# aarchiiive/diff-unet-amos

Measured on AMD Instinct MI355X. Metric: denoised voxel-steps/sec on 96^3 16-class AMOS patches, higher is better.
Workload: dtype f16

## Files before the change

diff_unet_amos_amd/csrc/conv3_args.hpp:

```cpp
#pragma once
#include "common.hpp"

namespace dua {

struct Conv3Args {
  const void* x; const void* w; const float* bias; void* y;
  stat_t* stats;
  InXform xf;
  int N, D, H, W;
  int Cin, Cin_stride, Cin_off;
  int Cout, Cout_stride, Cout_off;
  int nchunks, ntiles, tiles_h, tiles_w, cout_pad;
  int ksplit, units_per_split;
  float* part;
  int tap_ch;
  int in_blk, out_blk;
  const void* bw_raw; int bw_stride, bw_off;
  InXform bw_xf;
  double* bw_sums;
};

int launch_conv3_wide(Conv3Args a, int D, hipStream_t s, bool persistent, int stagger = 0);
bool conv3_wide_takes_bwd_sums(const Conv3Args& a);

}
```

diff_unet_amos_amd/csrc/conv3d_igemm.hip:

```cpp
#include "common.hpp"
#include "../../include/dua_hip.h"
#include "conv3_args.hpp"
#include "stamp.hpp"
#include <algorithm>

namespace dua {

namespace c3 {
constexpr int TD = 4, TH = 8, TW = 8;
constexpr int HD = TD + 2, HH = TH + 2, HW = TW + 2;
constexpr int KG = 4;
constexpr int VS = KG * 16;
constexpr int RS = HW * VS + 16;
constexpr int PS = HH * RS;
constexpr int HALO_BYTES = HD * PS;
constexpr int BN = 64;
}

static inline int conv_variant_of(const dua_conv3_desc* d) { return d->policy & 0xff; }
static inline bool conv_policy_ok(const dua_conv3_desc* d) {
  const int v = d->policy & 0xff;
  return (d->policy & ~(0xff | DUA_POLICY_NO_FINISH)) == 0 && (v == 0 || v == 2 || v == 3 || v == 6 || v == 7 || v == 8 || v == 9);
}

#ifdef DUA_ABLATE
extern int g_wgrad_abl;
#endif

namespace c3v2 {
using namespace c3;
constexpr int SLAB = 3 * KG * BN * 16;
constexpr int LDS_MAIN = HALO_BYTES + 2 * SLAB;
}

__device__ __forceinline__ void glds16(const void* g, void* lds_wave_base) {
  __builtin_amdgcn_global_load_lds((const __attribute__((address_space(1))) void*)g,
                                   (__attribute__((address_space(3))) void*)lds_wave_base, 16, 0, 0);
}

template <typename T, int TDP = 4, int NKS = 2, bool HALF = false, bool BIG = false>
__global__ __launch_bounds__(256, BIG ? 1 : 2) void conv3d_k3_v2_kernel(Conv3Args a) {
  using namespace c3v2;
  constexpr int TD = TDP, HD = TDP + 2, MB = TDP == 2 ? 1 : 2;
  constexpr int NW = 4, NTHR = 64 * NW;
  constexpr int BSLAB = 3 * SLAB;
  constexpr int HALO_BYTES = HD * PS, LDS_MAIN = HALO_BYTES + (BIG ? 3 * BSLAB : 2 * SLAB);
  static_assert(!BIG || (NKS == 2 && !HALF), "the kd-plane form is the plain 32-channel-chunk kernel");
  constexpr int NITEMS = HD * HH * HW * KG, NIT = (NITEMS + NTHR - 1) / NTHR;
  constexpr int NPIECE = SLAB / 16, NSL = (NPIECE + NTHR - 1) / NTHR;
  using Frag = typename Elem<T>::Frag;
  constexpr int EPG = Elem<T>::EPG;
  constexpr int CK = KG * EPG;
  extern __shared__ __attribute__((aligned(16))) char smem[];
  char* halo = smem;
  char* wbuf = smem + HALO_BYTES;
  float* xsc = (float*)(smem + LDS_MAIN);
  float* xsh = xsc + a.nchunks * CK;
  float* xad = xsh + a.nchunks * CK;

  const int tid = threadIdx.x, lane = tid & 63, wave = tid >> 6;
  const int r = lane & 31, hh = lane >> 5;
  const int dwave = TDP == 2 ? wave >> 1 : wave;
  const int hbase = TDP == 2 ? (wave & 1) * 4 : 0;
  const int tile = xcd_remap(blockIdx.x, a.ntiles);
  const int ct = blockIdx.y, n = blockIdx.z % a.N;
  const int tw_ = tile % a.tiles_w, th_ = (tile / a.tiles_w) % a.tiles_h, td_ = tile / (a.tiles_w * a.tiles_h);
  const int d0 = td_ * TD, h0 = th_ * TH, w0 = tw_ * TW;
  const bool fused = a.xf.stats != nullptr;

  const int kg_t = tid & (KG - 1);
  long goff[NIT]; int loff[NIT];
  const T* xin = (const T*)a.x + (long)n * a.D * a.H * a.W * a.Cin_stride + a.Cin_off;
#pragma unroll
  for (int j = 0; j < NIT; ++j) {
    int it = tid + NTHR * j;
// ... 710 lines not shown
#pragma unroll
      for (int e = 0; e < 4; ++e) {
        o[e] = (T)acc[e];
        const float f = (float)o[e];
        s[e] += f; q[e] += (part_t)f * (part_t)f;
      }
      if (c < Cout) {
        T* yp = y + ((long)n * vox + v) * Cout_stride + Cout_off + c;
#pragma unroll
        for (int e = 0; e < 4; ++e) yp[e] = o[e];
      }
    }
  }
#pragma unroll
  for (int e = 0; e < 4; ++e) { red[threadIdx.x][e] = s[e]; red[threadIdx.x][4 + e] = q[e]; }
  __syncthreads();
  for (int ch = threadIdx.x; ch < 4 * G; ch += 256) {
    const int g4 = ch >> 2, e = ch & 3;
    double S = 0, Q = 0;
    for (int j = 0; j < VL; ++j) { S += (double)red[j * G + g4][e]; Q += (double)red[j * G + g4][4 + e]; }
    if (ch < Cout) stats_add(stats, n, cout_pad, blockIdx.x & (STAT_REPLICAS - 1), ch, S, Q);
  }
}


static inline void choose_split(int base_wgs, int units, int* ksplit, int* ups, int target = 320, int max_base = 64) {
  *ksplit = 1; *ups = units;
  if (base_wgs > max_base || units <= 1) return;
  int want = target == 320 ? (320 + base_wgs - 1) / base_wgs : target / base_wgs;
  if (want < 1) want = 1;
  if (want > units) want = units;
  *ups = (units + want - 1) / want;
  *ksplit = (units + *ups - 1) / *ups;
}

constexpr int PARTIAL_LDS_PAD = 36 * 1024;

static const LdsAttr kConvLdsAttrs[] = {
    {(const void*)conv3d_k3_v2_kernel<f16, 4>, c3v2::LDS_MAIN + 3 * 4 * 1024 + PARTIAL_LDS_PAD},
    {(const void*)conv3d_k3_v2_kernel<float, 4>, c3v2::LDS_MAIN + 3 * 4 * 1024 + PARTIAL_LDS_PAD},
    {(const void*)conv3d_k3_v2_kernel<f16, 4, 1>, c3v2::LDS_MAIN + 4096 + PARTIAL_LDS_PAD},
    {(const void*)conv3d_k3_v2_kernel<f16, 4, 0>, c3v2::LDS_MAIN + 4096 + PARTIAL_LDS_PAD},
    {(const void*)conv3d_k3_v2_kernel<f16, 4, 2, true>, c3v2::LDS_MAIN + 3 * 4 * 1024 + PARTIAL_LDS_PAD},
    {(const void*)conv3d_k3_first_kernel, c3f::LDS_F + 2048 + PARTIAL_LDS_PAD},
    {(const void*)conv3d_k3_v2_kernel<f16, 2>, c3v2::LDS_MAIN + 3 * 4 * 1024},
    {(const void*)conv3d_k3_v2_kernel<float, 2>, c3v2::LDS_MAIN + 3 * 4 * 1024},
    {(const void*)conv3d_k3_v2_kernel<f16, 4, 2, false, true>, 160 * 1024},
    {(const void*)conv3d_k3_v2_kernel<float, 4, 2, false, true>, 160 * 1024},
    {(const void*)conv3d_k3_v2_kernel<f16, 2, 2, false, true>, 160 * 1024},
    {(const void*)conv3d_k3_v2_kernel<float, 2, 2, false, true>, 160 * 1024},
};
static const LdsAttrs kConvLdsReg(kConvLdsAttrs);

static int conv3_kernel_kind(const dua_conv3_desc* d, bool fused) {
  const int g_conv_variant = conv_variant_of(d);
  if (d->dtype != DUA_F16) return 0;
  if (d->tap_channel_plus1 > 0) return (d->tap_channel_plus1 == 17 && g_conv_variant == 0) ? 1 : 0;
  const long tiles = (long)((d->D + 3) / 4) * ((d->H + 7) / 8) * ((d->W + 7) / 8) * ((d->Cout + c3::BN - 1) / c3::BN) * d->N;
  const long vox = (long)d->D * d->H * d->W;
  if ((g_conv_variant == 0 || g_conv_variant == 8 || g_conv_variant == 9) && !d->background && tiles >= 1024 && d->D % 8 == 0 && d->H % 8 == 0 && d->W % 8 == 0 &&
      d->Cin % 16 == 0 && d->Cin <= (fused ? 256 : 384) && vox * d->Cin_stride < 0x7fffffffL)
    return 2;
  return 0;
}

struct BwdSums { const void* raw; int stride, off; const dua_in_norm* in; double* sums; };

template <typename T>
static int launch_conv3(const dua_conv3_desc* d, const void* x, const void* w, const float* bias,
                        const dua_in_norm* in, void* y, stat_t* stats, float* ws, long ws_bytes, hipStream_t s,
                        const BwdSums* bw = nullptr) {
  using namespace c3;
  constexpr int CK = KG * Elem<T>::EPG;
  Conv3Args a;
  a.x = x; a.w = w; a.bias = bias; a.y = y; a.stats = stats;
  a.bw_raw = nullptr; a.bw_stride = a.bw_off = 0; a.bw_xf = make_xform(nullptr, d->Cout); a.bw_sums = nullptr;
  if (bw) {
    a.bw_raw = bw->raw; a.bw_stride = bw->stride; a.bw_off = bw->off; a.bw_xf = make_xform(bw->in, d->Cout); a.bw_sums = bw->sums;
  }
  a.xf = make_xform(in, d->Cin);
  a.N = d->N; a.D = d->D; a.H = d->H; a.W = d->W;
  a.Cin = d->Cin; a.Cin_stride = d->Cin_stride; a.Cin_off = d->Cin_off;
  a.Cout = d->Cout; a.Cout_stride = d->Cout_stride; a.Cout_off = d->Cout_off;
  a.nchunks = (d->Cin + CK - 1) / CK;
  const int td = (d->D + TD - 1) / TD;
  a.tiles_h = (d->H + TH - 1) / TH; a.tiles_w = (d->W + TW - 1) / TW;
  a.ntiles = td * a.tiles_h * a.tiles_w;
  const int nct = (d->Cout + BN - 1) / BN;
  a.cout_pad = nct * BN;
  a.ksplit = 1; a.units_per_split = a.nchunks * 3; a.part = nullptr; a.tap_ch = -1;
  a.in_blk = d->layout & DUA_IN_BLOCKED ? 1 : 0; a.out_blk = d->layout & DUA_OUT_BLOCKED ? 1 : 0;
  if (a.nchunks * CK > 1024 || !conv_policy_ok(d)) return DUA_ERR_ARG;
  const int g_conv_variant = conv_variant_of(d);
  const int kind = conv3_kernel_kind(d, in && in->stats);
  if ((a.in_blk && kind != 2) || (a.out_blk && kind == 0)) return DUA_ERR_ARG;
  if ((a.in_blk && (d->Cin_off % 16 || d->Cin_stride % 16)) || (a.out_blk && (d->Cout_off % 16 || d->Cout_stride % 16))) return DUA_ERR_ARG;
  const int xf_bytes = in && in->stats ? 3 * 4 * a.nchunks * CK : 0;
  if (int e = ensure_prepared()) return e;
  const long vox = (long)d->D * d->H * d->W;
  const int bg_pad = d->background ? PARTIAL_LDS_PAD : 0;
  if (d->tap_channel_plus1 > 0) {
    a.tap_ch = d->tap_channel_plus1 - 1;
    if constexpr (sizeof(T) != 2) return DUA_ERR_ARG;
    else {
      if (a.nchunks != 1 || (in && in->stats) || (a.tap_ch != 0 && a.tap_ch != 16) || d->Cin != a.tap_ch + 8) return DUA_ERR_ARG;
      dim3 grid(a.ntiles, nct, d->N);
      if (kind == 1) {
        const int cus = device_cus();
        if (cus <= 0) return DUA_ERR_ARG;
        const int items = a.ntiles * d->N;
        const int wgs = std::max(1, (bg_pad ? 1 : 2) * cus / nct);
        hipLaunchKernelGGL(conv3d_k3_first_kernel, dim3(std::min(items, wgs), nct, 1), dim3(256), c3f::LDS_F + 2048 + bg_pad, s, a, items);
        return (int)hipGetLastError();
      }
      if (a.tap_ch == 16) hipLaunchKernelGGL((conv3d_k3_v2_kernel<T, 4, 1>), grid, dim3(256), c3v2::LDS_MAIN + 4096 + bg_pad, s, a);
      else hipLaunchKernelGGL((conv3d_k3_v2_kernel<T, 4, 0>), grid, dim3(256), c3v2::LDS_MAIN + 4096 + bg_pad, s, a);
      return (int)hipGetLastError();
    }
  }
  if constexpr (sizeof(T) == 2) {
    if (kind == 2) return launch_conv3_wide(a, d->D, s, g_conv_variant >= 8, g_conv_variant == 9 ? 2 : 0);
  }
  if (bw) return DUA_ERR_ARG;
  const bool autop = g_conv_variant == 0 || g_conv_variant == 2 || g_conv_variant == 6 || g_conv_variant == 7 || g_conv_variant >= 8;
  const bool big = g_conv_variant == 0 || g_conv_variant == 2 || g_conv_variant == 7 || g_conv_variant >= 8;
  if (ws != nullptr && autop) {
    int ks, ups;
    if (g_conv_variant == 2) choose_split(a.ntiles * nct * d->N, a.nchunks * 3, &ks, &ups, 512, 256);
    else choose_split(a.ntiles * nct * d->N, a.nchunks * 3, &ks, &ups, big ? 256 : 320);
    if (ks > 1 && (long)ks * d->N * vox * a.cout_pad * 4 <= ws_bytes) { a.ksplit = ks; a.units_per_split = ups; a.part = ws; }
  }
  if (a.ksplit == 1 && ((autop && a.ntiles * nct * d->N < 200 && a.ntiles * nct * d->N > 64) || g_conv_variant == 3)) {
    const int td2 = (d->D + 1) / 2;
    a.ntiles = td2 * a.tiles_h * a.tiles_w;
    dim3 grid2(a.ntiles, nct, d->N);
    constexpr int LDS2 = 4 * c3::HH * c3::RS + 2 * c3v2::SLAB;
    const bool big2 = big && (long)a.ntiles * nct * d->N <= 256;
    if (big2) hipLaunchKernelGGL((conv3d_k3_v2_kernel<T, 2, 2, false, true>), grid2, dim3(256), 4 * c3::HH * c3::RS + 9 * c3v2::SLAB + xf_bytes, s, a);
    else hipLaunchKernelGGL((conv3d_k3_v2_kernel<T, 2>), grid2, dim3(256), LDS2 + xf_bytes, s, a);
    return (int)hipGetLastError();
  }
  dim3 grid(a.ntiles, nct, d->N * a.ksplit);
  if (a.ksplit > 1) {
    if (big) hipLaunchKernelGGL((conv3d_k3_v2_kernel<T, 4, 2, false, true>), grid, dim3(256), c3::HALO_BYTES + 9 * c3v2::SLAB + xf_bytes, s, a);
    else hipLaunchKernelGGL(conv3d_k3_v2_kernel<T>, grid, dim3(256), c3v2::LDS_MAIN + xf_bytes, s, a);
    if (d->policy & DUA_POLICY_NO_FINISH) return (int)hipGetLastError();
    const int G = a.cout_pad / 4 > 256 ? 256 : a.cout_pad / 4;
    if (a.cout_pad / 4 > 256) return DUA_ERR_ARG;
    const int VL = 256 / G;
    int ITER = 8;
    while (ITER > 1 && (vox + (long)VL * ITER - 1) / ((long)VL * ITER) < 128) ITER >>= 1;
    dim3 fgrid((unsigned)((vox + (long)VL * ITER - 1) / ((long)VL * ITER)), d->N);
    hipLaunchKernelGGL(splitk_finish_kernel<T>, fgrid, dim3(256), 0, s, (const float*)ws, a.ksplit, d->N, vox, a.cout_pad,
                       d->Cout, bias, (T*)y, d->Cout_stride, d->Cout_off, stats, G, VL, ITER);
    return (int)hipGetLastError();
  }
  if (sizeof(T) == 2 && d->Cin - (a.nchunks - 1) * CK <= CK / 2)
    hipLaunchKernelGGL((conv3d_k3_v2_kernel<T, 4, 2, true>), grid, dim3(256), c3v2::LDS_MAIN + xf_bytes + bg_pad, s, a);
  else
    hipLaunchKernelGGL(conv3d_k3_v2_kernel<T>, grid, dim3(256), c3v2::LDS_MAIN + xf_bytes + bg_pad, s, a);
  return (int)hipGetLastError();
}

}

extern "C" {

#ifdef DUA_STAMP
long dua_debug_stamps(void* host, long bytes) { return dua::stamps_out(host, bytes); }
#endif

#ifdef DUA_ABLATE
int dua_set_option(int key, int value) {
  if (key == 3 && value >= 0 && value < 16) { dua::g_wgrad_abl = value; return 0; }
  return DUA_ERR_ARG;
}
#endif

int dua_conv3d_k3_kernel_kind(const dua_conv3_desc* d, int fused, int has_workspace) {
  if (!d || !dua::conv_policy_ok(d)) return DUA_ERR_ARG;
  (void)has_workspace;
  return dua::conv3_kernel_kind(d, fused != 0);
}

long dua_conv3d_k3_workspace(const dua_conv3_desc* d) {
  using namespace dua::c3;
  if (!d || (d->dtype != DUA_F16 && d->dtype != DUA_F32)) return DUA_ERR_ARG;
  const int ck = 4 * (d->dtype == DUA_F16 ? 8 : 4);
  const int nch = (d->Cin + ck - 1) / ck, nct = (d->Cout + BN - 1) / BN;
  const int tiles = ((d->D + TD - 1) / TD) * ((d->H + TH - 1) / TH) * ((d->W + TW - 1) / TW);
  int ks, ups;
  dua::choose_split(tiles * nct * d->N, nch * 3, &ks, &ups);
  return ks > 1 ? (long)ks * d->N * d->D * d->H * d->W * nct * BN * 4 : 0;
}

int dua_conv3d_k3_fwd(const dua_conv3_desc* d, const void* x, const void* w_packed, const float* bias_padded,
                      const dua_in_norm* in, void* y, dua_stat_word* out_stats, void* workspace, long workspace_bytes,
                      void* stream) {
  if (!d || !x || !w_packed || !bias_padded || !y || !out_stats) return DUA_ERR_ARG;
  if (d->Cin % 8 || d->Cout % 8 || d->Cin_stride % 8 || d->Cout_stride % 8 || d->Cin_off % 8 || d->Cout_off % 8)
    return DUA_ERR_ARG;
  if (in && in->stats && (!in->gamma || !in->beta || in->c_pad < d->Cin || in->count <= 0 || !(in->slope >= 0.f && in->slope <= 1.f))) return DUA_ERR_ARG;
  if (d->dtype == DUA_F16)
    return dua::launch_conv3<dua::f16>(d, x, w_packed, bias_padded, in, y, out_stats, (float*)workspace, workspace_bytes, (hipStream_t)stream);
  if (d->dtype == DUA_F32)
    return dua::launch_conv3<float>(d, x, w_packed, bias_padded, in, y, out_stats, (float*)workspace, workspace_bytes, (hipStream_t)stream);
  return DUA_ERR_ARG;
}

int dua_conv3d_k3_dgrad_reduce_supported(const dua_conv3_desc* d) {
  if (!d || d->dtype != DUA_F16 || d->layout || d->tap_channel_plus1 || d->background || dua::conv_variant_of(d) != 0) return 0;
  return dua::conv3_kernel_kind(d, false) == 2 ? 1 : 0;
}

int dua_conv3d_k3_dgrad_reduce(const dua_conv3_desc* d, const void* dy, const void* w_packed, const float* bias_padded, void* dx,
                               const void* raw, int raw_stride, int raw_off, const dua_in_norm* raw_in, double* sums, void* stream) {
  if (!dua_conv3d_k3_dgrad_reduce_supported(d) || !dy || !w_packed || !bias_padded || !dx || !raw || !raw_in || !sums) return DUA_ERR_ARG;
  if (d->Cin % 8 || d->Cout % 8 || d->Cin_stride % 8 || d->Cout_stride % 8 || d->Cin_off % 8 || d->Cout_off % 8) return DUA_ERR_ARG;
  if (!raw_in->stats || !raw_in->gamma || !raw_in->beta || raw_in->c_pad < d->Cout || raw_in->count <= 0 ||
      !(raw_in->slope >= 0.f && raw_in->slope <= 1.f) || raw_stride % 8 || raw_off % 8 || raw_off + d->Cout > raw_stride)
    return DUA_ERR_ARG;
  const dua::BwdSums bw{raw, raw_stride, raw_off, raw_in, sums};
  return dua::launch_conv3<dua::f16>(d, dy, w_packed, bias_padded, nullptr, dx, nullptr, nullptr, 0, (hipStream_t)stream, &bw);
}

}
```

diff_unet_amos_amd/csrc/conv3d_wide.hip:

```cpp
#include "common.hpp"
#include "../../include/dua_hip.h"
#include "conv3_args.hpp"
#include "stamp.hpp"
#include "named_acc.hpp"

namespace dua {

namespace c3w {
constexpr int TH = 8, TW = 8, HH = TH + 2, HW = TW + 2;
constexpr int VSF = 32, RSF = 12 * VSF, PSF = HH * RSF;
constexpr int BN = 64;
constexpr int WPLANE = 18 * 1024;
constexpr int HALO_MAX = 10 * PSF;
constexpr int LDS_FIXED = HALO_MAX + 2 * WPLANE;
constexpr int SLAB = 3 * 4 * BN * 16;
}

__device__ __forceinline__ void dma_piece(const char* src_lane, unsigned lds_dst) {
  unsigned keep;
  asm volatile("s_mov_b32 %0, m0\n\ts_mov_b32 m0, %2\n\ts_nop 0\n\tglobal_load_lds_dwordx4 %1, off\n\ts_mov_b32 m0, %0"
               : "=&s"(keep) : "v"(src_lane), "s"(__builtin_amdgcn_readfirstlane(lds_dst)) : "memory");
}

#ifndef WIDE_LA
#define WIDE_LA 1
#endif
template <int MB, bool BWD = false>
__device__ __forceinline__ void wide_tile(const Conv3Args& a, char* smem, const int d0, const int h0, const int w0,
                                          const int ct, const int n, const int replica) {
  using namespace c3w;
  using T = f16;
  constexpr int TD = 2 * MB, HD = TD + 2, NH = MB / 2;
  char* halo = smem;
  char* wbuf = smem + HALO_MAX;
  float* xsc = (float*)(smem + LDS_FIXED);
  float* xsh = xsc + a.Cin;
  float* xad = xsh + a.Cin;

  const int tid = threadIdx.x, lane = tid & 63, wave = tid >> 6;
  const int r = lane & 31, hh = lane >> 5;
  const bool fused = a.xf.stats != nullptr;
  const int nhc = (a.Cin + 15) >> 4;
  const int U = nhc * 3;

  const int p_t = tid & 1, pos = tid >> 1;
  const int hy = pos / HW, hx = pos - hy * HW;
  const int gh = h0 + hy - 1, gw = w0 + hx - 1;
  const bool ok_hw = pos < HH * HW && (unsigned)gh < (unsigned)a.H && (unsigned)gw < (unsigned)a.W;
  const int vstride = a.in_blk ? 16 : a.Cin_stride;
  const long hcstride = a.in_blk ? (long)a.D * a.H * a.W * 16 : 16;
  const T* xin = (const T*)a.x + (long)n * a.D * a.H * a.W * a.Cin_stride + (a.in_blk ? (long)(a.Cin_off >> 4) * a.D * a.H * a.W * 16 : a.Cin_off) + p_t * 8;
  const int voff = ok_hw ? (((d0 - 1) * a.H + gh) * a.W + gw) * vstride : 0;
  const int pstep = a.H * a.W * vstride;
  const int loff = pos < HH * HW ? hy * RSF + hx * VSF + ((p_t ^ (hy & 1)) << 4) : HW * VSF + (p_t << 4);
  f16x8 hreg[HD];
  auto load_halo = [&](int hc, int j0, int j1) {
    const T* src = xin + hc * hcstride;
#pragma unroll
    for (int j = 0; j < HD; ++j) {
      if (j < j0 || j >= j1) continue;
      const bool dok = (unsigned)(d0 + j - 1) < (unsigned)a.D;
      hreg[j] = *(const f16x8*)(src + (ok_hw && dok ? voff + j * pstep : 0));
    }
  };
  auto store_halo = [&](int hc) {
    float sc[8], sh[8], ad[8], sn[8];
    if (fused) {
      const int c0 = hc * 16 + p_t * 8;
#pragma unroll
      for (int e = 0; e < 8; ++e) { sc[e] = xsc[c0 + e]; sh[e] = xsh[c0 + e]; ad[e] = xad[c0 + e]; }
      xform_prep<T>(sc, sh, ad, sn, a.xf.slope);
    }
#pragma unroll
    for (int j = 0; j < HD; ++j) {
      f16x8 v = hreg[j];
      if (fused) v = xform_frag<T>(v, sc, sh, ad, sn, a.xf.slope);
      const f32x4 raw = __builtin_bit_cast(f32x4, v);
      const bool ok = ok_hw && (unsigned)(d0 + j - 1) < (unsigned)a.D;
      f32x4 o;
#pragma unroll
      for (int e = 0; e < 4; ++e) o[e] = ok ? raw[e] : 0.f;
      *(f32x4*)(halo + loff + j * PSF) = o;
    }
  };

  const char* wsrc = (const char*)a.w + (long)ct * a.nchunks * 9 * SLAB + lane * 16;
  const unsigned wlds = (unsigned)(size_t)(__attribute__((address_space(3))) char*)wbuf;
  auto dma_plane = [&](int u, int slot) {
    const int hc = u / 3, kd = u - hc * 3;
    const char* src = wsrc + (long)((hc >> 1) * 3 + kd) * 3 * SLAB + (hc & 1) * 2048;
#pragma unroll
    for (int j = 0; j < 5; ++j) {
      const int p = wave + 4 * j;
      if (p < 18) dma_piece(src + ((p >> 1) * 4 + (p & 1)) * 1024, wlds + slot * WPLANE + p * 1024);
    }
  };

  DUA_STAMP_AT(0, true);
  DUA_STAMP_AT(2, false);
  float bias_q[2];
#pragma unroll
  for (int q = 0; q < 2; ++q) {
    const int bc = ct * BN + q * 32 + r;
    bias_q[q] = bc >= a.Cout ? 0.f : a.bias[bc];
  }
  constexpr int UN = 4;
  stat_t sv[UN][2 * STAT_WORDS];
  float gam[UN], bet[UN], addv[UN];
  if (fused) {
    const int part = lane >> 4;
#pragma unroll
    for (int u = 0; u < UN; ++u) {
      const int c = (wave + 4 * u) * 16 + (lane & 15), cc = c < a.Cin ? c : a.Cin - 1;
      gam[u] = a.xf.gamma[cc]; bet[u] = a.xf.beta[cc];
      addv[u] = a.xf.add ? a.xf.add[(long)n * a.xf.add_stride + cc] : 0.f;
      const stat_t* sp = a.xf.stats + ((long)n * STAT_REPLICAS + 2 * part) * STAT_WORDS * a.xf.c_pad + cc;
      if ((wave + 4 * u) * 16 < a.Cin) {
#pragma unroll
        for (int k = 0; k < 2 * STAT_WORDS; ++k) sv[u][k] = sp[(long)k * a.xf.c_pad];
      } else {
#pragma unroll
        for (int k = 0; k < 2 * STAT_WORDS; ++k) sv[u][k] = 0;
      }
    }
  }
  float* bwc = (float*)(smem + LDS_FIXED) + (fused ? 3 * a.Cin : 0);
  double bwS = 0, bwQ = 0;
  float bwg = 0.f, bwb = 0.f;
  constexpr bool bwd = BWD;
  if (bwd) {
    const int c = ct * BN + wave * 16 + (lane & 15), cc = c < a.Cout ? c : a.Cout - 1;
    bwg = a.bw_xf.gamma[cc]; bwb = a.bw_xf.beta[cc];
    stats_read_wave16(a.bw_xf.stats, n, a.bw_xf.c_pad, cc, bwS, bwQ);
  }
  DUA_STAMP_AT(56, false);
  load_halo(0, 0, HD);
  DUA_STAMP_AT(57, false);
  dma_plane(0, 0);
  DUA_STAMP_AT(59, false);
  if (fused) {
    const int part = lane >> 4;
    double Sm = 0, Qm = 0;
    float gm = 0.f, bm = 0.f, am = 0.f;
#pragma unroll
    for (int u = 0; u < UN; ++u) {
      stat_t w[STAT_WORDS];
#pragma unroll
      for (int k = 0; k < STAT_WORDS; ++k) {
        w[k] = sv[u][k] + sv[u][STAT_WORDS + k];
        w[k] += __shfl_xor(w[k], 16);
        w[k] += __shfl_xor(w[k], 32);
      }
      if (part == u) {
        Sm = (double)w[0] + (double)w[1] * (1.0 / STAT_FRAC);
        Qm = (double)w[2] + (double)w[3] * (1.0 / STAT_FRAC);
        gm = gam[u]; bm = bet[u]; am = addv[u];
      }
    }
    const int c = (wave + 4 * part) * 16 + (lane & 15);
    const double mean = Sm * a.xf.inv_count;
    double var = Qm * a.xf.inv_count - mean * mean;
    var = var > 0 ? var : 0;
    const float g = gm * (float)(1.0 / sqrt(var + (double)a.xf.eps));
    if (c < a.Cin) {
      xsc[c] = g;
      xsh[c] = bm - (float)mean * g;
      xad[c] = am;
    }
    __syncthreads();
  }
  if (bwd && lane < 16) {
    const double mean = bwS * a.bw_xf.inv_count;
    double var = bwQ * a.bw_xf.inv_count - mean * mean;
    var = var > 0 ? var : 0;
    const int cl = wave * 16 + lane;
    bwc[cl] = (float)mean;
    bwc[64 + cl] = (float)(1.0 / sqrt(var + (double)a.bw_xf.eps));
    bwc[128 + cl] = bwg;
    bwc[192 + cl] = bwb;
  }
  DUA_STAMP_AT(60, false);
  DUA_STAMP_AT(61, false);
  store_halo(0);
  const int dsl = MB == 4 ? 2 * wave : wave;
  f32x16 acc[MB][2];
#pragma unroll
  for (int q = 0; q < 2; ++q)
#pragma unroll
    for (int m = 0; m < MB; ++m)
#pragma unroll
      for (int i = 0; i < 16; ++i) acc[m][q][i] = bias_q[q];
  asm volatile("s_waitcnt vmcnt(0)" ::: "memory");
  __syncthreads();
  DUA_STAMP_AT(3, false);

  const int sw = (r >> 3) & 1;
  const int a_base = dsl * PSF + (r >> 3) * RSF + (r & 7) * VSF;
  const int a_even = a_base + ((hh ^ sw) << 4), a_odd = a_base + ((hh ^ sw ^ 1) << 4);
  const int b_base = (hh * BN + r) * 16;

  auto phase = [&](int kd, int slot) __attribute__((always_inline)) {
    const char* hp = halo + kd * PSF;
    const char* wb = wbuf + slot * WPLANE + b_base;
    f16x8 fa[WIDE_LA + 1][2], fb[2][2];
    auto ldA = [&](int t, int sub, int b) {
      const int kh = t / 3, kw = t - kh * 3;
      const char* ap = hp + ((kh & 1) ? a_odd : a_even) + sub * PSF + kh * RSF + kw * VSF;
      fa[b][0] = *(const f16x8*)ap;
      fa[b][1] = *(const f16x8*)(ap + 4 * RSF);
    };
    auto ldB = [&](int t, int b) {
      fb[b][0] = *(const f16x8*)(wb + t * 2048);
      fb[b][1] = *(const f16x8*)(wb + t * 2048 + 512);
    };
    ldB(0, 0);
#pragma unroll
    for (int h = 0; h < WIDE_LA; ++h) ldA(h / NH, h % NH, h);
#pragma unroll
    for (int h = 0; h < 9 * NH; ++h) {
      const int t = h / NH, sub = h % NH;
      if (h + WIDE_LA < 9 * NH) {
        const int t1 = (h + WIDE_LA) / NH, sub1 = (h + WIDE_LA) % NH;
        if (WIDE_LA == 1 && sub1 == 0) ldB(t1, t1 & 1);
        ldA(t1, sub1, (h + WIDE_LA) % (WIDE_LA + 1));
      }
      if (WIDE_LA > 1 && sub == 0 && t + 1 < 9) ldB(t + 1, (t + 1) & 1);
      __builtin_amdgcn_sched_barrier(0);
      mma32(acc[2 * sub][0], fa[h % (WIDE_LA + 1)][0], fb[t & 1][0]);
      mma32(acc[2 * sub][1], fa[h % (WIDE_LA + 1)][0], fb[t & 1][1]);
      mma32(acc[2 * sub + 1][0], fa[h % (WIDE_LA + 1)][1], fb[t & 1][0]);
      mma32(acc[2 * sub + 1][1], fa[h % (WIDE_LA + 1)][1], fb[t & 1][1]);
      __builtin_amdgcn_sched_barrier(0);
    }
  };

  constexpr int J1 = HD == 10 ? 4 : 2, J2 = HD == 10 ? 7 : 4;
  for (int hc = 0; hc < nhc; ++hc) {
    const bool more = hc + 1 < nhc;
#pragma unroll
    for (int kd = 0; kd < 3; ++kd) {
      const int u = hc * 3 + kd, slot = u & 1;
      if (u + 1 < U) dma_plane(u + 1, slot ^ 1);
      if (more) load_halo(hc + 1, kd == 0 ? 0 : kd == 1 ? J1 : J2, kd == 0 ? J1 : kd == 1 ? J2 : HD);
      phase(kd, slot);
      if (more && kd == 0) asm volatile("s_waitcnt vmcnt(%0)" ::"n"(J1) : "memory");
      else if (more && kd == 1) asm volatile("s_waitcnt vmcnt(%0)" ::"n"(J2 - J1) : "memory");
      else asm volatile("s_waitcnt vmcnt(0)" ::: "memory");
      __syncthreads();
      if (u < 26) DUA_STAMP_AT(4 + u, false);
    }
    if (more) {
      store_halo(hc + 1);
      if (hc < 7) DUA_STAMP_AT(30 + 2 * hc, false);
      __syncthreads();
      if (hc < 7) DUA_STAMP_AT(31 + 2 * hc, false);
    }
  }
  DUA_STAMP_AT(62, false);

  char* ot = halo + wave * 8192;
  float* ex = (float*)wbuf;
  const long nvox = (long)a.D * a.H * a.W;
  T* yout = (T*)a.y + (long)n * nvox * a.Cout_stride;
  float s[2] = {0.f, 0.f}, ss[2] = {0.f, 0.f};
  if (bwd) {
    const int cg = lane & 7;
    float m8[8], r8[8], g8[8], b8[8], s0[8], s1[8], s2[8];
#pragma unroll
    for (int e = 0; e < 8; ++e) {
      m8[e] = bwc[cg * 8 + e]; r8[e] = bwc[64 + cg * 8 + e]; g8[e] = bwc[128 + cg * 8 + e]; b8[e] = bwc[192 + cg * 8 + e];
      s0[e] = s1[e] = s2[e] = 0.f;
    }
    const float slope = a.bw_xf.slope;
    const T* rawn = (const T*)a.bw_raw + (long)n * nvox * a.bw_stride + a.bw_off + ct * BN + cg * 8;
    const bool cok = ct * BN + cg * 8 < a.Cout;
#pragma unroll
    for (int pr = 0; pr < MB / 2; ++pr) {
      const int gd = d0 + dsl + pr;
      f16x8 yv[8];
#pragma unroll
      for (int it = 0; it < 8; ++it) {
        const int v = it * 8 + (lane >> 3);
        const long vx = ((long)gd * a.H + h0 + (v >> 3)) * a.W + w0 + (v & 7);
        yv[it] = *(const f16x8*)(rawn + (cok ? vx * a.bw_stride : 0));
      }
#pragma unroll
      for (int mm = 0; mm < 2; ++mm)
#pragma unroll
        for (int q = 0; q < 2; ++q)
#pragma unroll
          for (int i = 0; i < 16; ++i)
            *(T*)(ot + mm * 4096 + acc_row(i, hh) * 128 + (q * 32 + r) * 2) = (T)acc[2 * pr + mm][q][i];
      __builtin_amdgcn_fence(__ATOMIC_RELEASE, "wavefront");
      __builtin_amdgcn_wave_barrier();
      __builtin_amdgcn_fence(__ATOMIC_ACQUIRE, "wavefront");
#pragma unroll
      for (int it = 0; it < 8; ++it) {
// ... 49 lines not shown
  for (int pr = 0; pr < MB / 2; ++pr) {
#pragma unroll
    for (int mm = 0; mm < 2; ++mm)
#pragma unroll
      for (int q = 0; q < 2; ++q)
#pragma unroll
        for (int i = 0; i < 16; ++i) {
          const float v = acc[2 * pr + mm][q][i];
          s[q] += v;
          ss[q] = fmaf(v, v, ss[q]);
          *(T*)(ot + mm * 4096 + acc_row(i, hh) * 128 + (q * 32 + r) * 2) = (T)v;
        }
    __builtin_amdgcn_fence(__ATOMIC_RELEASE, "wavefront");
    __builtin_amdgcn_wave_barrier();
    __builtin_amdgcn_fence(__ATOMIC_ACQUIRE, "wavefront");
    const int gd = d0 + dsl + pr;
#pragma unroll
    for (int it = 0; it < 8; ++it) {
      const int v = it * 8 + (lane >> 3), cg = lane & 7;
      const int gh = h0 + (v >> 3), gw = w0 + (v & 7);
      if (ct * BN + cg * 8 < a.Cout)
        *(f16x8*)(yout + chan_off(a.out_blk, ((long)gd * a.H + gh) * a.W + gw, a.Cout_off + ct * BN + cg * 8, a.Cout_stride, nvox)) =
            *(const f16x8*)(ot + v * 128 + cg * 16);
    }
    __builtin_amdgcn_fence(__ATOMIC_RELEASE, "wavefront");
    __builtin_amdgcn_wave_barrier();
    __builtin_amdgcn_fence(__ATOMIC_ACQUIRE, "wavefront");
  }
#pragma unroll
  for (int q = 0; q < 2; ++q) {
    s[q] += __shfl_xor(s[q], 32);
    ss[q] += __shfl_xor(ss[q], 32);
    if (hh == 0) { ex[(wave * BN + q * 32 + r) * 2] = s[q]; ex[(wave * BN + q * 32 + r) * 2 + 1] = ss[q]; }
  }
  __syncthreads();
  if (wave == 0) {
    double S = 0, Q = 0;
#pragma unroll
    for (int w = 0; w < 4; ++w) { S += (double)ex[(w * BN + lane) * 2]; Q += (double)ex[(w * BN + lane) * 2 + 1]; }
    if (ct * BN + lane < a.Cout) stats_add(a.stats, n, a.cout_pad, replica, ct * BN + lane, S, Q);
  }
  DUA_STAMP_AT(63, false);
  DUA_STAMP_AT(1, true);
}

__global__ __launch_bounds__(256, 2) void conv3d_k3_wide_kernel(Conv3Args a) {
  extern __shared__ __attribute__((aligned(16))) char smem[];
  const int per_slab = a.tiles_h * a.tiles_w;
  const int tile = xcd_remap(blockIdx.x, a.ntiles);
  const int td = tile / per_slab, rem = tile - td * per_slab, th = rem / a.tiles_w, tw = rem - th * a.tiles_w;
  wide_tile<4>(a, smem, td * 8, th * 8, tw * 8, blockIdx.y, blockIdx.z, blockIdx.x & (STAT_REPLICAS - 1));
}


__global__ __launch_bounds__(256, 2) void conv3d_k3_wide_bwd_kernel(Conv3Args a) {
  extern __shared__ __attribute__((aligned(16))) char smem[];
  const int per_slab = a.tiles_h * a.tiles_w;
  const int tile = xcd_remap(blockIdx.x, a.ntiles);
  const int td = tile / per_slab, rem = tile - td * per_slab, th = rem / a.tiles_w, tw = rem - th * a.tiles_w;
  wide_tile<4, true>(a, smem, td * 8, th * 8, tw * 8, blockIdx.y, blockIdx.z, blockIdx.x & (STAT_REPLICAS - 1));
}

__global__ __launch_bounds__(256, 2) DUA_NAMED_ACC_KERNEL void conv3d_k3_wide_pt_kernel(Conv3Args a) {
  using namespace c3w;
  using T = f16;
  extern __shared__ __attribute__((aligned(16))) char smem[];
  char* halo = smem;
  char* wbuf = smem + HALO_MAX;
  float* xsc = (float*)(smem + LDS_FIXED);
  float* xsh = xsc + a.Cin;
  float* xad = xsh + a.Cin;
  float* ex = xad + (a.xf.stats ? a.Cin : 0) - (a.xf.stats ? 0 : 2 * a.Cin);
  constexpr int HD = 10;

  const int tid = threadIdx.x, lane = tid & 63, wave = __builtin_amdgcn_readfirstlane(tid >> 6);
  const int r = lane & 31, hh = lane >> 5;
  const int ct = blockIdx.y, n = blockIdx.z, replica = blockIdx.x & (STAT_REPLICAS - 1);
  const bool fused = a.xf.stats != nullptr;
  const int nhc = (a.Cin + 15) >> 4;
  const int per_slab = a.tiles_h * a.tiles_w;

  const int p_t = tid & 1, pos = tid >> 1;
  const int hy = pos / HW, hx = pos - hy * HW;
  const int vstride = a.in_blk ? 16 : a.Cin_stride;
  const long hcstride = a.in_blk ? (long)a.D * a.H * a.W * 16 : 16;
  const T* xin = (const T*)a.x + (long)n * a.D * a.H * a.W * a.Cin_stride + (a.in_blk ? (long)(a.Cin_off >> 4) * a.D * a.H * a.W * 16 : a.Cin_off) + p_t * 8;
  const int pstep = a.H * a.W * vstride;
  const int loff = pos < HH * HW ? hy * RSF + hx * VSF + ((p_t ^ (hy & 1)) << 4) : HW * VSF + (p_t << 4);
  f16x8 hreg[HD];
  struct Geo { int d0, h0, w0, voff; bool ok_hw; };
  auto geo_of = [&](int t) {
    Geo g;
    const int tile = xcd_remap(t, a.ntiles);
    const int td = tile / per_slab, rem = tile - td * per_slab, th = rem / a.tiles_w, tw = rem - th * a.tiles_w;
    g.d0 = td * 8; g.h0 = th * 8; g.w0 = tw * 8;
    const int gh = g.h0 + hy - 1, gw = g.w0 + hx - 1;
    g.ok_hw = pos < HH * HW && (unsigned)gh < (unsigned)a.H && (unsigned)gw < (unsigned)a.W;
    g.voff = g.ok_hw ? (((g.d0 - 1) * a.H + gh) * a.W + gw) * vstride : 0;
    return g;
  };
  auto load_halo = [&](const Geo& g, int hc, int j0, int j1) {
    const T* src = xin + hc * hcstride;
#pragma unroll
    for (int j = 0; j < HD; ++j) {
      if (j < j0 || j >= j1) continue;
      const bool dok = (unsigned)(g.d0 + j - 1) < (unsigned)a.D;
// ... 166 lines not shown
        __builtin_amdgcn_fence(__ATOMIC_ACQUIRE, "wavefront");
        const int gd = cur.d0 + 2 * wave + pr;
#pragma unroll
        for (int it = 0; it < 8; ++it) {
          const int v = it * 8 + (lane >> 3), cg = lane & 7;
          const int gh = cur.h0 + (v >> 3), gw = cur.w0 + (v & 7);
          if (ct * BN + cg * 8 < a.Cout)
            *(f16x8*)(yout + chan_off(a.out_blk, ((long)gd * a.H + gh) * a.W + gw, a.Cout_off + ct * BN + cg * 8, a.Cout_stride, nvox)) =
                *(const f16x8*)(ot + v * 128 + cg * 16);
        }
        __builtin_amdgcn_fence(__ATOMIC_RELEASE, "wavefront");
        __builtin_amdgcn_wave_barrier();
        __builtin_amdgcn_fence(__ATOMIC_ACQUIRE, "wavefront");
      }
#pragma unroll
      for (int q = 0; q < 2; ++q) { Sacc[q] += (double)s[q]; Qacc[q] += (double)ss[q]; }
    }
    if (!has_next) break;
    __syncthreads();
    t = tn;
    cur = nxt;
  }

  double* exd = (double*)(smem);
  __syncthreads();
#pragma unroll
  for (int q = 0; q < 2; ++q) {
    const double S = Sacc[q] + __shfl_xor(Sacc[q], 32), Q = Qacc[q] + __shfl_xor(Qacc[q], 32);
    if (hh == 0) { exd[(wave * BN + q * 32 + r) * 2] = S; exd[(wave * BN + q * 32 + r) * 2 + 1] = Q; }
  }
  __syncthreads();
  if (wave == 0) {
    double S = 0, Q = 0;
#pragma unroll
    for (int w = 0; w < 4; ++w) { S += exd[(w * BN + lane) * 2]; Q += exd[(w * BN + lane) * 2 + 1]; }
    if (ct * BN + lane < a.Cout) stats_add(a.stats, n, a.cout_pad, replica, ct * BN + lane, S, Q);
  }
  (void)ex;
}

static const LdsAttr kWideLdsAttrs[] = {{(const void*)conv3d_k3_wide_kernel, 80 * 1024}, {(const void*)conv3d_k3_wide_pt_kernel, 80 * 1024},
                                        {(const void*)conv3d_k3_wide_bwd_kernel, 80 * 1024}};
static const LdsAttrs kWideLdsReg(kWideLdsAttrs);

#ifdef DUA_STAMP
extern "C" long dua_debug_stamps_wide(void* host, long bytes) { return stamps_out(host, bytes); }
#endif

bool conv3_wide_takes_bwd_sums(const Conv3Args& a) {
  return a.bw_raw && a.bw_xf.stats && a.bw_xf.gamma && a.bw_xf.beta && a.bw_xf.c_pad >= a.Cout && a.bw_stride % 8 == 0 && a.bw_off % 8 == 0 &&
         (long)a.D * a.H * a.W * a.bw_stride < 0x7fffffffL;
}

int launch_conv3_wide(Conv3Args a, int D, hipStream_t s, bool persistent, int stagger) {
  using namespace c3w;
  if (int e = ensure_prepared()) return e;
  if (D % 8 || a.H % 8 || a.W % 8 || a.Cin % 16 || (a.xf.stats && a.Cin > 256)) return DUA_ERR_ARG;
  if (a.in_blk && (a.Cin_off % 16 || a.Cin_stride % 16)) return DUA_ERR_ARG;
  if (a.out_blk && (a.Cout_off % 16 || a.Cout_stride % 16)) return DUA_ERR_ARG;
  a.tiles_h = a.H / 8; a.tiles_w = a.W / 8;
  a.ntiles = (D / 8) * a.tiles_h * a.tiles_w;
  const int lds = LDS_FIXED + (a.xf.stats ? 3 * 4 * a.Cin : 0) + (a.bw_sums ? 1024 : 0);
  if (lds > 80 * 1024) return DUA_ERR_ARG;
  if (a.bw_sums && (persistent || !conv3_wide_takes_bwd_sums(a))) return DUA_ERR_ARG;
  if (persistent) {
    const int cus = device_cus();
    if (cus <= 0) return DUA_ERR_ARG;
    const int pairs = (a.cout_pad / BN) * a.N;
    int gx = (2 * cus + pairs - 1) / pairs;
    gx = (gx + 7) & ~7;
    if (gx > a.ntiles) gx = a.ntiles;
    a.ksplit = stagger;
    hipLaunchKernelGGL(conv3d_k3_wide_pt_kernel, dim3(gx, a.cout_pad / BN, a.N), dim3(256), lds, s, a);
    return (int)hipGetLastError();
  }
  if (a.bw_sums) hipLaunchKernelGGL(conv3d_k3_wide_bwd_kernel, dim3(a.ntiles, a.cout_pad / BN, a.N), dim3(256), lds, s, a);
  else hipLaunchKernelGGL(conv3d_k3_wide_kernel, dim3(a.ntiles, a.cout_pad / BN, a.N), dim3(256), lds, s, a);
  return (int)hipGetLastError();
}

}
```

Baseline: 675.2 million.

## Add single-round wide conv kernel with double-buffered halo and deeper weight ring

Adds a single-round variant of the wide 8x8x8 conv3d tile kernel for small-Cout layers whose tile count fits in one wave of CUs. It runs at one block per CU and uses static LDS holding two halo buffers and a four-slot weight-plane ring. Next-chunk halo loads, transforms and stores, plus weight DMAs, are interleaved inside the MMA loop through hooks, with fine-grained vmcnt waits in place of full drains. This targets exposed load latency where occupancy is low, at the cost of more LDS, half the occupancy and more complex wait accounting. Kernel selection for the default variant routes Cout<=48 layers with few enough tiles to this path.

```diff
diff --git a/diff_unet_amos_amd/csrc/conv3_args.hpp b/diff_unet_amos_amd/csrc/conv3_args.hpp
--- a/diff_unet_amos_amd/csrc/conv3_args.hpp
+++ b/diff_unet_amos_amd/csrc/conv3_args.hpp
@@ -20,7 +20,7 @@
   double* bw_sums;
 };
 
-int launch_conv3_wide(Conv3Args a, int D, hipStream_t s, bool persistent, int stagger = 0);
+int launch_conv3_wide(Conv3Args a, int D, hipStream_t s, bool persistent, int stagger = 0, bool single_round = false);
 bool conv3_wide_takes_bwd_sums(const Conv3Args& a);
 
 }
diff --git a/diff_unet_amos_amd/csrc/conv3d_igemm.hip b/diff_unet_amos_amd/csrc/conv3d_igemm.hip
--- a/diff_unet_amos_amd/csrc/conv3d_igemm.hip
+++ b/diff_unet_amos_amd/csrc/conv3d_igemm.hip
@@ -20,7 +20,7 @@
 static inline int conv_variant_of(const dua_conv3_desc* d) { return d->policy & 0xff; }
 static inline bool conv_policy_ok(const dua_conv3_desc* d) {
   const int v = d->policy & 0xff;
-  return (d->policy & ~(0xff | DUA_POLICY_NO_FINISH)) == 0 && (v == 0 || v == 2 || v == 3 || v == 6 || v == 7 || v == 8 || v == 9);
+  return (d->policy & ~(0xff | DUA_POLICY_NO_FINISH)) == 0 && (v == 0 || v == 2 || v == 3 || v == 6 || v == 7 || v == 8 || v == 9 || v == 10 || v == 11);
 }
 
 #ifdef DUA_ABLATE
@@ -837,15 +837,21 @@
 };
 static const LdsAttrs kConvLdsReg(kConvLdsAttrs);
 
+static constexpr long SR_MIN_TILES = 128, SR_MAX_COUT = 48;
 static int conv3_kernel_kind(const dua_conv3_desc* d, bool fused) {
   const int g_conv_variant = conv_variant_of(d);
   if (d->dtype != DUA_F16) return 0;
   if (d->tap_channel_plus1 > 0) return (d->tap_channel_plus1 == 17 && g_conv_variant == 0) ? 1 : 0;
   const long tiles = (long)((d->D + 3) / 4) * ((d->H + 7) / 8) * ((d->W + 7) / 8) * ((d->Cout + c3::BN - 1) / c3::BN) * d->N;
   const long vox = (long)d->D * d->H * d->W;
-  if ((g_conv_variant == 0 || g_conv_variant == 8 || g_conv_variant == 9) && !d->background && tiles >= 1024 && d->D % 8 == 0 && d->H % 8 == 0 && d->W % 8 == 0 &&
-      d->Cin % 16 == 0 && d->Cin <= (fused ? 256 : 384) && vox * d->Cin_stride < 0x7fffffffL)
-    return 2;
+  const bool wide_ok = !d->background && d->D % 8 == 0 && d->H % 8 == 0 && d->W % 8 == 0 && d->Cin % 16 == 0 &&
+                       d->Cin <= (fused ? 256 : 384) && vox * d->Cin_stride < 0x7fffffffL;
+  if ((g_conv_variant == 0 || g_conv_variant >= 8) && wide_ok && tiles >= 1024) return 2;
+  const long tiles8 = vox / 512;
+  if (((g_conv_variant == 0 && d->Cout <= SR_MAX_COUT) || g_conv_variant == 11) && wide_ok && tiles8 >= SR_MIN_TILES &&
+      ensure_prepared() == 0 && device_cus() > 0 &&
+      tiles8 * ((d->Cout + c3::BN - 1) / c3::BN) * d->N <= device_cus())
+    return 3;
   return 0;
 }
 
@@ -878,7 +884,7 @@
   if (a.nchunks * CK > 1024 || !conv_policy_ok(d)) return DUA_ERR_ARG;
   const int g_conv_variant = conv_variant_of(d);
   const int kind = conv3_kernel_kind(d, in && in->stats);
-  if ((a.in_blk && kind != 2) || (a.out_blk && kind == 0)) return DUA_ERR_ARG;
+  if ((a.in_blk && kind != 2 && kind != 3) || (a.out_blk && kind == 0)) return DUA_ERR_ARG;
   if ((a.in_blk && (d->Cin_off % 16 || d->Cin_stride % 16)) || (a.out_blk && (d->Cout_off % 16 || d->Cout_stride % 16))) return DUA_ERR_ARG;
   const int xf_bytes = in && in->stats ? 3 * 4 * a.nchunks * CK : 0;
   if (int e = ensure_prepared()) return e;
@@ -904,7 +910,8 @@
     }
   }
   if constexpr (sizeof(T) == 2) {
-    if (kind == 2) return launch_conv3_wide(a, d->D, s, g_conv_variant >= 8, g_conv_variant == 9 ? 2 : 0);
+    if (kind == 2) return launch_conv3_wide(a, d->D, s, g_conv_variant == 8 || g_conv_variant == 9, g_conv_variant == 9 ? 2 : 0);
+    if (kind == 3) return launch_conv3_wide(a, d->D, s, false, 0, true);
   }
   if (bw) return DUA_ERR_ARG;
   const bool autop = g_conv_variant == 0 || g_conv_variant == 2 || g_conv_variant == 6 || g_conv_variant == 7 || g_conv_variant >= 8;
@@ -965,7 +972,8 @@
 int dua_conv3d_k3_kernel_kind(const dua_conv3_desc* d, int fused, int has_workspace) {
   if (!d || !dua::conv_policy_ok(d)) return DUA_ERR_ARG;
   (void)has_workspace;
-  return dua::conv3_kernel_kind(d, fused != 0);
+  const int kind = dua::conv3_kernel_kind(d, fused != 0);
+  return kind == 3 ? 2 : kind;
 }
 
 long dua_conv3d_k3_workspace(const dua_conv3_desc* d) {
diff --git a/diff_unet_amos_amd/csrc/conv3d_wide.hip b/diff_unet_amos_amd/csrc/conv3d_wide.hip
--- a/diff_unet_amos_amd/csrc/conv3d_wide.hip
+++ b/diff_unet_amos_amd/csrc/conv3d_wide.hip
@@ -1,3 +1,4 @@
+#include <type_traits>
 #include "common.hpp"
 #include "../../include/dua_hip.h"
 #include "conv3_args.hpp"
@@ -14,6 +15,8 @@
 constexpr int HALO_MAX = 10 * PSF;
 constexpr int LDS_FIXED = HALO_MAX + 2 * WPLANE;
 constexpr int SLAB = 3 * 4 * BN * 16;
+constexpr int SR_RING = 4;
+constexpr int LDS_FIXED_SR = 2 * HALO_MAX + SR_RING * WPLANE;
 }
 
 __device__ __forceinline__ void dma_piece(const char* src_lane, unsigned lds_dst) {
@@ -22,18 +25,35 @@
                : "=&s"(keep) : "v"(src_lane), "s"(__builtin_amdgcn_readfirstlane(lds_dst)) : "memory");
 }
 
+__device__ __forceinline__ void wait_vm(int n) {
+  switch (n) {
+#define DUA_WAIT_VM_CASE(k) case k: asm volatile("s_waitcnt vmcnt(" #k ")" ::: "memory"); break;
+    DUA_WAIT_VM_CASE(0) DUA_WAIT_VM_CASE(1) DUA_WAIT_VM_CASE(2) DUA_WAIT_VM_CASE(3) DUA_WAIT_VM_CASE(4) DUA_WAIT_VM_CASE(5)
+    DUA_WAIT_VM_CASE(6) DUA_WAIT_VM_CASE(7) DUA_WAIT_VM_CASE(8) DUA_WAIT_VM_CASE(9) DUA_WAIT_VM_CASE(10) DUA_WAIT_VM_CASE(11)
+    DUA_WAIT_VM_CASE(12) DUA_WAIT_VM_CASE(13) DUA_WAIT_VM_CASE(14) DUA_WAIT_VM_CASE(15) DUA_WAIT_VM_CASE(16) DUA_WAIT_VM_CASE(17)
+    DUA_WAIT_VM_CASE(18) DUA_WAIT_VM_CASE(19) DUA_WAIT_VM_CASE(20) DUA_WAIT_VM_CASE(21) DUA_WAIT_VM_CASE(22) DUA_WAIT_VM_CASE(23)
+    DUA_WAIT_VM_CASE(24) DUA_WAIT_VM_CASE(25) DUA_WAIT_VM_CASE(26) DUA_WAIT_VM_CASE(27) DUA_WAIT_VM_CASE(28) DUA_WAIT_VM_CASE(29)
+    DUA_WAIT_VM_CASE(30) DUA_WAIT_VM_CASE(31)
+#undef DUA_WAIT_VM_CASE
+    default: asm volatile("s_waitcnt vmcnt(0)" ::: "memory"); break;
+  }
+}
+
 #ifndef WIDE_LA
 #define WIDE_LA 1
 #endif
-template <int MB, bool BWD = false>
+template <int MB, bool BWD = false, bool SR = false>
 __device__ __forceinline__ void wide_tile(const Conv3Args& a, char* smem, const int d0, const int h0, const int w0,
                                           const int ct, const int n, const int replica) {
   using namespace c3w;
   using T = f16;
+  static_assert(!SR || (MB == 4 && !BWD), "single-round form: 8x8x8 tiles, forward epilogue");
   constexpr int TD = 2 * MB, HD = TD + 2, NH = MB / 2;
+  constexpr int RING = SR ? SR_RING : 2, NHB = SR ? 2 : 1;
+  constexpr int FIXED = NHB * HALO_MAX + RING * WPLANE;
   char* halo = smem;
-  char* wbuf = smem + HALO_MAX;
-  float* xsc = (float*)(smem + LDS_FIXED);
+  char* wbuf = smem + NHB * HALO_MAX;
+  float* xsc = (float*)(smem + FIXED);
   float* xsh = xsc + a.Cin;
   float* xad = xsh + a.Cin;
 
@@ -63,6 +83,25 @@
       hreg[j] = *(const f16x8*)(src + (ok_hw && dok ? voff + j * pstep : 0));
     }
   };
+  float psc[8], psh[8], pad[8], psn[8];
+  auto prep_halo = [&](int hc) {
+    if (fused) {
+      const int c0 = hc * 16 + p_t * 8;
+#pragma unroll
+      for (int e = 0; e < 8; ++e) { psc[e] = xsc[c0 + e]; psh[e] = xsh[c0 + e]; pad[e] = xad[c0 + e]; }
+      xform_prep<T>(psc, psh, pad, psn, a.xf.slope);
+    }
+  };
+  auto store_plane = [&](int j, char* hb) __attribute__((always_inline)) {
+    f16x8 v = hreg[j];
+    if (fused) v = xform_frag<T>(v, psc, psh, pad, psn, a.xf.slope);
+    const f32x4 raw = __builtin_bit_cast(f32x4, v);
+    const bool ok = ok_hw && (unsigned)(d0 + j - 1) < (unsigned)a.D;
+    f32x4 o;
+#pragma unroll
+    for (int e = 0; e < 4; ++e) o[e] = ok ? raw[e] : 0.f;
+    *(f32x4*)(hb + loff + j * PSF) = o;
+  };
   auto store_halo = [&](int hc) {
     float sc[8], sh[8], ad[8], sn[8];
     if (fused) {
@@ -124,7 +163,7 @@
       }
     }
   }
-  float* bwc = (float*)(smem + LDS_FIXED) + (fused ? 3 * a.Cin : 0);
+  float* bwc = (float*)(smem + FIXED) + (fused ? 3 * a.Cin : 0);
   double bwS = 0, bwQ = 0;
   float bwg = 0.f, bwb = 0.f;
   constexpr bool bwd = BWD;
@@ -137,6 +176,7 @@
   load_halo(0, 0, HD);
   DUA_STAMP_AT(57, false);
   dma_plane(0, 0);
+  if constexpr (SR) { dma_plane(1, 1); dma_plane(2, 2); }
   DUA_STAMP_AT(59, false);
   if (fused) {
     const int part = lane >> 4;
@@ -190,7 +230,9 @@
     for (int m = 0; m < MB; ++m)
 #pragma unroll
       for (int i = 0; i < 16; ++i) acc[m][q][i] = bias_q[q];
-  asm volatile("s_waitcnt vmcnt(0)" ::: "memory");
+  const int P = __builtin_amdgcn_readfirstlane(wave) < 2 ? 5 : 4;
+  if constexpr (SR) wait_vm(2 * P);
+  else asm volatile("s_waitcnt vmcnt(0)" ::: "memory");
   __syncthreads();
   DUA_STAMP_AT(3, false);
 
@@ -199,8 +241,8 @@
   const int a_even = a_base + ((hh ^ sw) << 4), a_odd = a_base + ((hh ^ sw ^ 1) << 4);
   const int b_base = (hh * BN + r) * 16;
 
-  auto phase = [&](int kd, int slot) __attribute__((always_inline)) {
-    const char* hp = halo + kd * PSF;
+  auto phase = [&](int kd, int slot, const char* hbuf, auto&& hook) __attribute__((always_inline)) {
+    const char* hp = hbuf + kd * PSF;
     const char* wb = wbuf + slot * WPLANE + b_base;
     f16x8 fa[WIDE_LA + 1][2], fb[2][2];
     auto ldA = [&](int t, int sub, int b) {
@@ -231,10 +273,42 @@
       mma32(acc[2 * sub + 1][0], fa[h % (WIDE_LA + 1)][1], fb[t & 1][0]);
       mma32(acc[2 * sub + 1][1], fa[h % (WIDE_LA + 1)][1], fb[t & 1][1]);
       __builtin_amdgcn_sched_barrier(0);
-    }
-  };
+      if constexpr (SR) {
+        hook(h);
+        __builtin_amdgcn_sched_barrier(0);
+      }
+    }
+  };
+  auto no_hook = [](int) {};
 
   constexpr int J1 = HD == 10 ? 4 : 2, J2 = HD == 10 ? 7 : 4;
+  if constexpr (SR) {
+    auto half_chunk = [&](int hc, auto more_c) __attribute__((always_inline)) {
+      constexpr bool MORE = decltype(more_c)::value;
+      char* hcur = halo + (hc & 1) * HALO_MAX;
+      char* hnext = halo + ((hc + 1) & 1) * HALO_MAX;
+#pragma unroll
+      for (int kd = 0; kd < 3; ++kd) {
+        const int u = hc * 3 + kd;
+        phase(kd, u % RING, hcur, [&](int h) __attribute__((always_inline)) {
+          if constexpr (MORE) {
+            if (kd < 2 && h == 0) dma_plane(u + RING - 1, (u + RING - 1) % RING);
+            if (kd == 2 && h == 17) dma_plane(u + RING - 1, (u + RING - 1) % RING);
+            if (kd < 2 && h % 3 == 1 && h <= 13) load_halo(hc + 1, kd * 5 + h / 3, kd * 5 + h / 3 + 1);
+            if (kd >= 1 && h == 6) prep_halo(hc + 1);
+            if (kd >= 1 && h >= 7 && h < 12) store_plane((kd - 1) * 5 + h - 7, hnext);
+          }
+        });
+        const int c_cur = MORE ? (kd < 2 ? P + 5 : P) : 0;
+        const int c_prev = kd == 0 ? P : MORE ? P + 5 : 0;
+        wait_vm(kd == 2 && !MORE ? 0 : c_cur + c_prev);
+        __syncthreads();
+        if (u < 26) DUA_STAMP_AT(4 + u, false);
+      }
+    };
+    for (int hc = 0; hc + 1 < nhc; ++hc) half_chunk(hc, std::true_type{});
+    half_chunk(nhc - 1, std::false_type{});
+  } else
   for (int hc = 0; hc < nhc; ++hc) {
     const bool more = hc + 1 < nhc;
 #pragma unroll
@@ -242,7 +316,7 @@
       const int u = hc * 3 + kd, slot = u & 1;
       if (u + 1 < U) dma_plane(u + 1, slot ^ 1);
       if (more) load_halo(hc + 1, kd == 0 ? 0 : kd == 1 ? J1 : J2, kd == 0 ? J1 : kd == 1 ? J2 : HD);
-      phase(kd, slot);
+      phase(kd, slot, halo, no_hook);
       if (more && kd == 0) asm volatile("s_waitcnt vmcnt(%0)" ::"n"(J1) : "memory");
       else if (more && kd == 1) asm volatile("s_waitcnt vmcnt(%0)" ::"n"(J2 - J1) : "memory");
       else asm volatile("s_waitcnt vmcnt(0)" ::: "memory");
@@ -398,6 +472,13 @@
   wide_tile<4>(a, smem, td * 8, th * 8, tw * 8, blockIdx.y, blockIdx.z, blockIdx.x & (STAT_REPLICAS - 1));
 }
 
+__global__ __launch_bounds__(256, 1) void conv3d_k3_wide_sr_kernel(Conv3Args a) {
+  __shared__ __attribute__((aligned(16))) char smem[c3w::LDS_FIXED_SR + 3 * 4 * 256];
+  const int per_slab = a.tiles_h * a.tiles_w;
+  const int tile = xcd_remap(blockIdx.x, a.ntiles);
+  const int td = tile / per_slab, rem = tile - td * per_slab, th = rem / a.tiles_w, tw = rem - th * a.tiles_w;
+  wide_tile<4, false, true>(a, smem, td * 8, th * 8, tw * 8, blockIdx.y, blockIdx.z, blockIdx.x & (STAT_REPLICAS - 1));
+}
 
 __global__ __launch_bounds__(256, 2) void conv3d_k3_wide_bwd_kernel(Conv3Args a) {
   extern __shared__ __attribute__((aligned(16))) char smem[];
@@ -670,7 +751,7 @@
          (long)a.D * a.H * a.W * a.bw_stride < 0x7fffffffL;
 }
 
-int launch_conv3_wide(Conv3Args a, int D, hipStream_t s, bool persistent, int stagger) {
+int launch_conv3_wide(Conv3Args a, int D, hipStream_t s, bool persistent, int stagger, bool single_round) {
   using namespace c3w;
   if (int e = ensure_prepared()) return e;
   if (D % 8 || a.H % 8 || a.W % 8 || a.Cin % 16 || (a.xf.stats && a.Cin > 256)) return DUA_ERR_ARG;
@@ -678,6 +759,11 @@
   if (a.out_blk && (a.Cout_off % 16 || a.Cout_stride % 16)) return DUA_ERR_ARG;
   a.tiles_h = a.H / 8; a.tiles_w = a.W / 8;
   a.ntiles = (D / 8) * a.tiles_h * a.tiles_w;
+  if (single_round) {
+    if (persistent || a.bw_sums) return DUA_ERR_ARG;
+    hipLaunchKernelGGL(conv3d_k3_wide_sr_kernel, dim3(a.ntiles, a.cout_pad / BN, a.N), dim3(256), 0, s, a);
+    return (int)hipGetLastError();
+  }
   const int lds = LDS_FIXED + (a.xf.stats ? 3 * 4 * a.Cin : 0) + (a.bw_sums ? 1024 : 0);
   if (lds > 80 * 1024) return DUA_ERR_ARG;
   if (a.bw_sums && (persistent || !conv3_wide_takes_bwd_sums(a))) return DUA_ERR_ARG;
```

Result: no change. 674.9 million, median of 6 (-0.0%).
